# Anaesthesiaye/sound_event_detection_transformer

Hardware: AMD Instinct MI355X
Metric: audio clips/sec training throughput (B=64, 10s@64-mel) (higher is better)
Workload: dtype bf16; 1 GPU; URBAN-SED SEDT enc_layers=3 dec_at num_queries=10 B=64/GPU, 10 s @ 64-mel (B,1,500,64), full train step: fwd + Hungarian matching (device) + SetCriterion + bwd + clip 0.1 + AdamW, dropout 0.1; global_batch=64, parallelism=dp1

## Files before the change

### include/sedt_hip.h

```cpp
#ifndef SEDT_HIP_H
#define SEDT_HIP_H
#include <stddef.h>
#include <stdint.h>

#ifdef __cplusplus
extern "C" {
#endif

#define SEDT_F32 0
#define SEDT_BF16 1
#define SEDT_BF16X3 2

#define SEDT_ACT_NONE 0
#define SEDT_ACT_RELU 1
#define SEDT_ACT_SIGMOID 2

const char* sedt_last_error(void);
int sedt_version(void);

typedef struct SedtIgemm {
  int32_t M, N, K;
  const void* A;
  const void* B;
  int64_t lda, ldb;
// ... 19 lines not shown
  float* slab;
  int32_t tile_m, tile_n;
  float* colsum_out;
  uint8_t* bits_out;
  int64_t ldbits;
  int32_t mask_bits;
  int32_t f32ep;
  int32_t omap;
  int32_t o_Hi, o_Wi, o_sh, o_sw, o_h0, o_w0;
  int32_t btap_on;
  int32_t btap[8];
  void* split_out;
  int32_t awrap;
  int32_t pad2_;
  const void* bfrag;
} SedtIgemm;

int sedt_igemm(const SedtIgemm* args, int dtype, void* stream);
int sedt_sizeof(int which);
int sedt_igemm_group(const SedtIgemm* jobs, int njobs, int dtype, void* stream);
int sedt_wgrad_group(const SedtIgemm* jobs, int njobs, int dtype, void* stream);
int sedt_igemm_co(const SedtIgemm* main, const SedtIgemm* wjobs, int nw, int dtype, void* stream, int* taken);
int sedt_igemm_splitk(int M, int N, int K, int dtype);
int sedt_igemm_describe(const SedtIgemm* args, int dtype, int grouped, char* out, int cap);
int sedt_igemm_group_describe(const SedtIgemm* jobs, int njobs, int dtype, char* out, int cap);

int sedt_wgrad_reduce(const float* slab, int splitk, int R, int taps, int Ci, const float* rowscale,
                      float* out, void* stream);
int sedt_wgrad_reduce_bias(const float* slab, int splitk, int R, int taps, int Ci, const float* rowscale, float* out,
                           const float* colsum_slab, float* bias_out, void* stream);

typedef struct SedtPrefetch {
  const void* ptr[3];
  size_t bytes[3];
} SedtPrefetch;

typedef struct SedtSplitJob {
  const float* src;
  int64_t ld;
  void* dst;
  int32_t rows, cols, pattern;
  int32_t blk0;
} SedtSplitJob;
int sedt_split3(const SedtSplitJob* jobs, int njobs, void* stream);

#define SEDT_MAX_REDUCE_JOBS 40
// ... 324 lines not shown
```

### sound_event_detection_transformer_amd/csrc/host.cpp

```cpp
#include <math.h>
#include <stdint.h>
#include <vector>
#include "../../include/sedt_hip.h"

namespace sedt { void set_error(const char* fmt, ...); }

template <typename F>
static void lsa_rows_le_cols(int n, int m, F a, std::vector<int>& row_of_col) {
  const double INF = 1e300;
  std::vector<double> u(n + 1, 0.0), v(m + 1, 0.0), minv(m + 1);
  std::vector<int> p(m + 1, 0), way(m + 1, 0);
  std::vector<char> used(m + 1);
  for (int i = 1; i <= n; ++i) {
    p[0] = i;
    int j0 = 0;
    std::fill(minv.begin(), minv.end(), INF);
    std::fill(used.begin(), used.end(), 0);
    do {
      used[j0] = 1;
      int i0 = p[j0], j1 = 0;
      double delta = INF;
      for (int j = 1; j <= m; ++j) {
        if (used[j]) continue;
        double cur = a(i0 - 1, j - 1) - u[i0] - v[j];
// ... 44 lines not shown
        lsa_rows_le_cols(Q, n, [&](int q, int t) { return (double)c[(size_t)q * Nt + t]; }, roc);
        for (int t = 0; t < n; ++t)
          if (roc[t] >= 0) out[roc[t]] = t;
      }
    }
  }
  return 0;
}

extern "C" int sedt_sizeof(int which) {
  switch (which) {
    case 0: return (int)sizeof(SedtIgemm);
    case 1: return (int)sizeof(SedtReduceJob);
    case 2: return (int)sizeof(SedtSplitJob);
    case 3: return (int)sizeof(SedtPrefetch);
    case 4: return (int)sizeof(SedtCriterion);
    case 5: return (int)sizeof(SedtMatch);
    case 6: return (int)sizeof(SedtChunk);
    case 7: return (int)sizeof(SedtBnJob);
    case 8: return (int)sizeof(SedtPackJob);
    case 9: return (int)sizeof(SedtFragJob);
    case 10: return (int)sizeof(SedtPoolAt);
    case 11: return (int)sizeof(SedtCopyJob);
    default: return -1;
  }
}
```

### sound_event_detection_transformer_amd/csrc/igemm.hip

```cpp
#include <stdlib.h>
#include "common.h"

namespace sedt {

template <typename T> struct Cfg;
template <> struct Cfg<float> {
  static constexpr int BK = 32, PITCH = 33, EPC = 4, KSTEP = 2, UK = 1;
};
template <> struct Cfg<bf16_t> {
  static constexpr int BK = 64, PITCH = 72, EPC = 8, KSTEP = 16, UK = 4;
};

struct GatherGeom {
  int Hi, Wi, Ci, Ho, Wo, KH, KW, sh, sw, ph, pw, dh, dw, transposed;
};

__device__ __forceinline__ long gather_pix(const GatherGeom& g, int n, int ho, int wo, int kh, int kw) {
  int hi, wi;
  if (!g.transposed) {
    hi = ho * g.sh - g.ph + kh * g.dh;
    wi = wo * g.sw - g.pw + kw * g.dw;
    if ((unsigned)hi >= (unsigned)g.Hi || (unsigned)wi >= (unsigned)g.Wi) return -1;
  } else {
    int th = ho + g.ph - kh * g.dh, tw = wo + g.pw - kw * g.dw;
// ... 698 lines not shown
  int maxs = nkb / 4 > 1 ? nkb / 4 : 1;
  if (s > maxs) s = maxs;
  if (s > 128) s = 128;
  if (tiles <= 2) s = maxs < 512 ? maxs : 512;
  if (s < 1) s = 1;
  static int kslice = -1;
  if (kslice < 0) {
    const char* e = sedt::dev_getenv("SEDT_WGRAD_KSLICE");
    kslice = (e && e[0] == '1') ? 1 : 0;
  }
  if (kslice && dtype == SEDT_BF16) {
    const int taps = (N % 9 == 0 && (N / 9) % 64 == 0) ? 9 : 1;
    const double A = 2.0 * K * M, B = 2.0 * K * (N / taps);
    const double cur = (N > M ? 8.0 * A + B : A + 8.0 * B) + 2.0 * s * 4.0 * M * N;
    int s8 = ((s + 7) / 8) * 8;
    if (s8 < 8) s8 = 8;
    if (s8 <= maxs && s8 <= 128) {
      const double ks = A + B + 2.0 * s8 * 4.0 * M * N;
      if (ks < 0.8 * cur) s = s8;
    }
  }
  return s;
}
```

### sound_event_detection_transformer_amd/csrc/wgrad3.hip

```cpp
#include <stdlib.h>
#include <algorithm>
#include "wgrad3_body.h"

namespace sedt {

template <int BN>
__global__ __launch_bounds__(256) void wgrad3_kernel(const SedtIgemm p, const unsigned a_bytes, const unsigned b_bytes,
                                                     const int nmajor) {
  wgrad3_body<BN>(p, a_bytes, b_bytes, nmajor, blockIdx.x, blockIdx.y);
}

__global__ __launch_bounds__(256) void wgrad3_group_kernel(const WgradGroup g) { wgrad_group_run(g, blockIdx.x); }

template <int BN>
static int launch_wgrad3(const SedtIgemm& p, unsigned a_bytes, unsigned b_bytes, hipStream_t st) {
  SEDT_DESCRIBE("wgrad3_kernel<%d>", BN);
  constexpr size_t lds = (size_t)2 * (64 * ROWB + 64 * BN * 2);
  static bool attr_set = false;
  auto kern = wgrad3_kernel<BN>;
  if (!attr_set) {
    hipError_t e = hipFuncSetAttribute(reinterpret_cast<const void*>(kern), hipFuncAttributeMaxDynamicSharedMemorySize, (int)lds);
    if (e != hipSuccess) {
      set_error("wgrad3: hipFuncSetAttribute failed: %s", hipGetErrorString(e));
      return 1;
// ... 30 lines not shown
  long ab[WG_MAXG], bb[WG_MAXG];
  for (int base = 0; base < njobs; base += WG_MAXG) {
    const int n = std::min(WG_MAXG, njobs - base);
    for (int i = 0; i < n; ++i) {
      const SedtIgemm& p = jobs[base + i];
      if (!p.trans || wgrad_lds_envelope(p, &ab[i], &bb[i]) != 0 || !wgrad3_conv_ok(p)) return -1;
    }
  }
  static bool attr_set = false;
  constexpr size_t lds = (size_t)2 * (64 * ROWB + 64 * 64 * 2);
  if (!attr_set) {
    hipError_t e = hipFuncSetAttribute(reinterpret_cast<const void*>(wgrad3_group_kernel), hipFuncAttributeMaxDynamicSharedMemorySize,
                                       (int)lds);
    if (e != hipSuccess) {
      set_error("wgrad3 group: hipFuncSetAttribute failed: %s", hipGetErrorString(e));
      return 1;
    }
    attr_set = true;
  }
  for (int base = 0; base < njobs; base += WG_MAXG) {
    WgradGroup g, gw;
    g.n = gw.n = 0;
    const int n = std::min(WG_MAXG, njobs - base);
    int blk = 0;
    for (int j = 0; j < n; ++j) {
      const SedtIgemm& p = jobs[base + j];
      long a, b;
      wgrad_lds_envelope(p, &a, &b);
      if (wgrad4_ok(p)) {
        const int i = gw.n++;
        gw.p[i] = p;
        gw.a_bytes[i] = (unsigned)a;
        gw.b_bytes[i] = (unsigned)b;
        continue;
      }
      const int i = g.n++;
      g.p[i] = p;
      g.a_bytes[i] = (unsigned)a;
      g.b_bytes[i] = (unsigned)b;
      g.nwg[i] = ((p.N + 63) / 64) * ((p.M + 63) / 64);
      g.nmajor[i] = (p.N > p.M ? 1 : 0) + ((p.splitk >= 8 && p.splitk % 8 == 0) ? 2 : 0);
      g.blk0[i] = blk;
      blk += (g.nwg[i] * (p.splitk > 1 ? p.splitk : 1) + 7) / 8 * 8;
    }
    if (gw.n > 0)
      if (int r = launch_wgrad4_group(gw, st)) return r;
    if (g.n > 0) {
      g.blk0[g.n] = blk;
      hipLaunchKernelGGL(wgrad3_group_kernel, dim3(blk), dim3(256), lds, st, g);
// ... 50 lines not shown
  if ((p.M & 7) || (p.N & 7) || (p.lda & 7) || (p.ldb & 7)) return -1;
  if (!al16(p.A) || !al16(p.B)) return -1;
  if (p.conv && ((p.Ci & 7) || p.transposed)) return -1;
  long a_bytes = ((long)(p.K - 1) * p.lda + p.M) * 2;
  long b_rows = p.conv ? (long)((p.K + (long)p.Ho * p.Wo - 1) / ((long)p.Ho * p.Wo)) * p.Hi * p.Wi : (long)p.K;
  long b_bytes = ((b_rows - 1) * p.ldb + (p.conv ? p.Ci : p.N)) * 2;
  if (a_bytes >= (1L << 31) || b_bytes >= (1L << 31) || a_bytes <= 0 || b_bytes <= 0) return -1;
  *a_bytes_out = a_bytes;
  *b_bytes_out = b_bytes;
  return 0;
}

int wgrad_lds_try(const SedtIgemm& p, hipStream_t st) {
  long a_bytes, b_bytes;
  if (wgrad_lds_envelope(p, &a_bytes, &b_bytes) != 0) return -1;
  {
    int r3 = wgrad3_try(p, (unsigned)a_bytes, (unsigned)b_bytes, st);
    if (r3 >= 0) return r3;
  }
  return -1;
}

}
```

### sound_event_detection_transformer_amd/csrc/wgrad3_body.h

```cpp
#pragma once
#include "lds_gemm_common.h"

namespace sedt {

typedef __attribute__((ext_vector_type(4))) short w3_s16x4;
typedef __attribute__((ext_vector_type(8))) short w3_s16x8;
typedef __attribute__((address_space(3))) w3_s16x4 w3_lds_s16x4;

__device__ __forceinline__ int w3_uniform(int v) { return __builtin_amdgcn_readfirstlane(v); }

__device__ __forceinline__ int w3_swz(int row) {
  const int v = (row >> 1) & 7;
  return ((v & 1) << 2) | (v & 2) | (v >> 2);
}

template <int BN, bool CONV>
__device__ __forceinline__ void wgrad3_impl(const SedtIgemm& p, const unsigned a_bytes, const unsigned b_bytes, const int nmajor,
                                            const int bx, const int by) {
  constexpr int BM = 64, BKP = 64;
  constexpr int NI = BN / 64;
  constexpr int A_BYTES = BKP * ROWB;
  constexpr int B_ROWB = BN * 2;
  constexpr int STAGE_BYTES = A_BYTES + BKP * B_ROWB;
  constexpr int GA = 2, GB = BN / 32;
// ... 197 lines not shown
  float* out = p.splitk > 1 ? p.slab + (long)by * p.M * p.N : reinterpret_cast<float*>(p.C);
  const long ldo = p.splitk > 1 ? p.N : p.ldc;
#pragma unroll
  for (int j = 0; j < NI; ++j) {
    const int col = n0 + wn + j * 32 + (lane & 31);
    if (col < p.N) {
#pragma unroll
      for (int r = 0; r < 16; ++r) {
        const int row = m0 + wm + (r & 3) + 8 * (r >> 2) + 4 * (lane >> 5);
        if (row < p.M) out[(long)row * ldo + col] = acc[j][r];
      }
    }
  }
}

template <int BN>
__device__ __forceinline__ void wgrad3_body(const SedtIgemm& p, const unsigned a_bytes, const unsigned b_bytes, const int nmajor,
                                            const int bx, const int by) {
  if (p.conv) wgrad3_impl<BN, true>(p, a_bytes, b_bytes, nmajor, bx, by);
  else wgrad3_impl<BN, false>(p, a_bytes, b_bytes, nmajor, bx, by);
}

constexpr int WG_MAXG = 10;
struct WgradGroup {
  int n;
  int blk0[WG_MAXG + 1];
  int nwg[WG_MAXG];
  int nmajor[WG_MAXG];
  unsigned a_bytes[WG_MAXG], b_bytes[WG_MAXG];
  SedtIgemm p[WG_MAXG];
};

static_assert(sizeof(WgradGroup) <= 3900, "WgradGroup must fit the 4 KB kernel-argument segment");

__device__ __forceinline__ void wgrad_group_run(const WgradGroup& g, const int b) {
  int i = 0;
  while (i + 1 < g.n && b >= g.blk0[i + 1]) ++i;
  const int local = b - g.blk0[i];
  const int nwg = g.nwg[i], sk = g.p[i].splitk > 1 ? g.p[i].splitk : 1;
  if (local >= nwg * sk) return;
  if (g.nmajor[i] >= 2) {
    const int j = local >> 3;
    wgrad3_body<64>(g.p[i], g.a_bytes[i], g.b_bytes[i], g.nmajor[i], j % nwg, (local & 7) + 8 * (j / nwg));
  } else {
    wgrad3_body<64>(g.p[i], g.a_bytes[i], g.b_bytes[i], g.nmajor[i], local % nwg, local / nwg);
  }
}

}
```

### sound_event_detection_transformer_amd/csrc/wgrad4.hip

```cpp
#include <stdlib.h>
#include <algorithm>
#include "wgrad3_body.h"

namespace sedt {

__device__ __forceinline__ int w4_swz(int row) { return (row & 3) << 2; }

template <bool CONV, int S, int NA>
__device__ __forceinline__ void wgrad4_impl(const SedtIgemm& p, const unsigned a_bytes, const unsigned b_bytes, const int nmajor,
                                            const int bx, const int by) {
  constexpr int BM = 128 * NA, BN = 128, BKP = 64, NW = 8;
  constexpr int IMG_ROWB = 256;
  constexpr int IMG_BYTES = BKP * IMG_ROWB;
  constexpr int STAGE_BYTES = (NA + 1) * IMG_BYTES;
  constexpr int B_IMG = NA * IMG_BYTES;
  constexpr int CPR = 16, RPI = 4;
  constexpr int GB = BKP / RPI / NW, GA = NA * GB;
  constexpr int G = GA + GB;
  constexpr int MI = 2 * NA;
  constexpr unsigned OOB = 0x80000000u;
  extern __shared__ __attribute__((aligned(16))) unsigned char smem[];
  const int t = threadIdx.x, lane = t & 63;
  const int wave = w3_uniform(t >> 6);
  const int kgrp = wave >> 2;
// ... 275 lines not shown
  if (nmajor & 2) {
    if (p.conv) wgrad4_impl<true, 3, 2>(p, a_bytes, b_bytes, nmajor, bx, by);
    else wgrad4_impl<false, 3, 2>(p, a_bytes, b_bytes, nmajor, bx, by);
    return;
  }
  if (p.conv) wgrad4_impl<true, S, 1>(p, a_bytes, b_bytes, nmajor, bx, by);
  else wgrad4_impl<false, S, 1>(p, a_bytes, b_bytes, nmajor, bx, by);
}

template <int S>
__global__ __launch_bounds__(512) void wgrad4_kernel(const SedtIgemm p, const unsigned a_bytes, const unsigned b_bytes,
                                                     const int nmajor) {
  wgrad4_body<S>(p, a_bytes, b_bytes, nmajor, blockIdx.x, blockIdx.y);
}

template <int S>
__global__ __launch_bounds__(512) void wgrad4_group_kernel(const WgradGroup g) {
  const int b = blockIdx.x;
  int i = 0;
  while (i + 1 < g.n && b >= g.blk0[i + 1]) ++i;
  const int local = b - g.blk0[i];
  const int nwg = g.nwg[i], sk = g.p[i].splitk > 1 ? g.p[i].splitk : 1;
  if (local >= nwg * sk) return;
  wgrad4_body<S>(g.p[i], g.a_bytes[i], g.b_bytes[i], g.nmajor[i], local % nwg, local / nwg);
}

static int wg4_stages() {
  static int s = -1;
  if (s < 0) {
    const char* e = sedt::dev_getenv("SEDT_WGRAD4_STAGES");
    s = (e && atoi(e) == 3) ? 3 : (e && atoi(e) == 4) ? 4 : 3;
  }
  return s;
}
int wgrad4_tile_m(int M, int N) {
  static int bm = -1, min_tiles = 1;
  if (bm < 0) {
    const char* e = sedt::dev_getenv("SEDT_WGRAD4_BM");
    bm = (e && atoi(e) == 128) ? 128 : 256;
    e = sedt::dev_getenv("SEDT_WGRAD4_WIDE_MIN");
    min_tiles = e ? atoi(e) : 1;
  }
  return (bm == 256 && M % 256 == 0 && (long)(M / 256) * (N / 128) >= min_tiles) ? 256 : 128;
}
static size_t wg4_lds() {
  const size_t narrow = (size_t)wg4_stages() * 2 * 64 * 256, wide = (size_t)3 * 3 * 64 * 256;
  return wgrad4_tile_m(256, 1 << 20) == 256 ? std::max(narrow, wide) : narrow;
}

bool wgrad4_shape_ok(int M, int N) {
  static int mn = -1;
  if (mn < 0) {
    const char* e = sedt::dev_getenv("SEDT_WGRAD4_MIN");
    mn = e ? atoi(e) : 256;
  }
  return M >= mn && N >= mn && (M % 128) == 0 && (N % 128) == 0;
}

bool wgrad4_ok(const SedtIgemm& p) {
  static int on = -1;
  if (on < 0) {
    const char* e = sedt::dev_getenv("SEDT_WGRAD_V4");
    on = (e && e[0] == '0') ? 0 : 1;
  }
  static int with_bias = -1;
  if (with_bias < 0) {
    const char* e = sedt::dev_getenv("SEDT_WGRAD4_BIAS");
    with_bias = (e && e[0] == '1') ? 1 : 0;
  }
  return on && p.trans && wgrad4_shape_ok(p.M, p.N) && (p.colsum_out == nullptr || with_bias) && p.out_f32 &&
         (p.splitk > 1 ? p.slab != nullptr : ((p.ldc & 3) == 0 && (reinterpret_cast<uintptr_t>(p.C) & 15) == 0)) &&
         (reinterpret_cast<uintptr_t>(p.slab) & 15) == 0;
}

static bool wg4_cbmajor(const SedtIgemm& p) {
  static int on = -1;
  if (on < 0) {
    const char* e = sedt::dev_getenv("SEDT_WGRAD4_CBMAJOR");
    on = e ? atoi(e) : 1;
  }
  return on && p.conv && p.KH * p.KW > 1 && (p.Ci % 128) == 0 && p.N == p.KH * p.KW * p.Ci;
}

template <typename K>
static int wg4_attr(K kern, const char* what) {
  hipError_t e = hipFuncSetAttribute(reinterpret_cast<const void*>(kern), hipFuncAttributeMaxDynamicSharedMemorySize, (int)wg4_lds());
  if (e != hipSuccess) {
    set_error("%s: hipFuncSetAttribute failed: %s", what, hipGetErrorString(e));
    return 1;
  }
  return 0;
}

// ... 14 lines not shown
}

int launch_wgrad4_group(WgradGroup& g, hipStream_t st) {
  static bool attr_set = false;
  if (!attr_set) {
    if (wg4_attr(wgrad4_group_kernel<3>, "wgrad4 group") || wg4_attr(wgrad4_group_kernel<4>, "wgrad4 group")) return 1;
    attr_set = true;
  }
  int blk = 0;
  for (int i = 0; i < g.n; ++i) {
    const SedtIgemm& p = g.p[i];
    const int bm = wgrad4_tile_m(p.M, p.N);
    g.nwg[i] = (p.N / 128) * (p.M / bm);
    g.nmajor[i] = (p.N > p.M ? 1 : 0) | (bm == 256 ? 2 : 0) | (wg4_cbmajor(p) ? 4 : 0);
    g.blk0[i] = blk;
    blk += (g.nwg[i] * (p.splitk > 1 ? p.splitk : 1) + 7) / 8 * 8;
  }
  g.blk0[g.n] = blk;
  if (wg4_stages() == 4) hipLaunchKernelGGL(wgrad4_group_kernel<4>, dim3(blk), dim3(512), wg4_lds(), st, g);
  else hipLaunchKernelGGL(wgrad4_group_kernel<3>, dim3(blk), dim3(512), wg4_lds(), st, g);
  return check_launch("wgrad4_group");
}

}
```

### sound_event_detection_transformer_amd/lib.py

```python
import ctypes as C
import os

import torch

HERE = os.path.dirname(os.path.abspath(__file__))
LIB_PATH = os.path.join(HERE, 'libsedt_hip.so')
if os.environ.get('SEDT_LIB_AB') and os.environ.get('SEDT_DEV') == '1':
    LIB_PATH = os.environ['SEDT_LIB_AB']

F32, BF16 = 0, 1
BF16X3 = 2
GEMM_X3 = False


def gemm_dtype(dtype):
    return BF16X3 if (dtype == F32 and GEMM_X3) else dtype
ACT_NONE, ACT_RELU, ACT_SIGMOID = 0, 1, 2
TORCH_DTYPE = {F32: torch.float32, BF16: torch.bfloat16}


class SedtIgemm(C.Structure):
    _fields_ = [
        ('M', C.c_int32), ('N', C.c_int32), ('K', C.c_int32),
        ('A', C.c_void_p), ('B', C.c_void_p),
# ... 45 lines not shown
POOL_MODES = {'max': 0, 'avg': 1, 'attn': 2, 'weighted_sum': 3}


class SedtMatch(C.Structure):
    _fields_ = [(n, C.c_void_p) for n in ('logits', 'boxes', 'lab_cat', 'lab_off', 'box_cat', 'box_off', 'ratio_cat', 'tc',
                                           'coef', 'wbox', 'tbox', 'tidx', 'tgt_len', 'gt_weak', 'assign')] + \
               [(n, C.c_int32) for n in ('L', 'B', 'ns', 'Q', 'C', 'n_lab', 'max_targets')] + \
               [('layer_of', C.c_int32 * CRIT_MAXL), ('w_class', C.c_float), ('w_bbox', C.c_float), ('w_giou', C.c_float),
                ('fl', C.c_int32), ('fine_tune', C.c_int32), ('normalize', C.c_int32), ('alpha_fl', C.c_float),
                ('gamma_fl', C.c_float), ('epsilon', C.c_float), ('alpha', C.c_float), ('ft_rand', C.c_void_p),
                ('ft_seed', C.c_uint32), ('seed_ptr', C.c_void_p), ('split', C.c_void_p), ('Qs', C.c_int32), ('q0', C.c_int32)]


class SedtSplitJob(C.Structure):
    _fields_ = [('src', C.c_void_p), ('ld', C.c_int64), ('dst', C.c_void_p), ('rows', C.c_int32), ('cols', C.c_int32),
                ('pattern', C.c_int32), ('blk0', C.c_int32)]


class SedtCopyJob(C.Structure):
    _fields_ = [('src', C.c_void_p), ('dst', C.c_void_p), ('src_stride', C.c_int64), ('dst_stride', C.c_int64), ('outer', C.c_int32),
                ('inner', C.c_int32), ('blk0', C.c_int32), ('pad_', C.c_int32)]


class SedtPrefetch(C.Structure):
    _fields_ = [('ptr', C.c_void_p * 3), ('bytes', C.c_size_t * 3)]


def prefetch_arg(tensors):
    ts = [t for t in (tensors or ()) if t is not None][:3]
    if not ts:
        return None
    a = SedtPrefetch()
    for i, t in enumerate(ts):
        a.ptr[i], a.bytes[i] = t.data_ptr(), t.numel() * t.element_size()
    return C.byref(a)


MAX_REDUCE_JOBS = 40
_vp, _i, _i64, _f, _d, _u32, _sz = C.c_void_p, C.c_int, C.c_int64, C.c_float, C.c_double, C.c_uint32, C.c_size_t

SIGNATURES = {
    'sedt_last_error': (C.c_char_p, []),
    'sedt_version': (_i, []),
    'sedt_sizeof': (_i, [_i]),
    'sedt_igemm': (_i, [C.POINTER(SedtIgemm), _i, _vp]),
    'sedt_igemm_group': (_i, [C.POINTER(SedtIgemm), _i, _i, _vp]),
    'sedt_wgrad_group': (_i, [C.POINTER(SedtIgemm), _i, _i, _vp]),
    'sedt_igemm_co': (_i, [C.POINTER(SedtIgemm), C.POINTER(SedtIgemm), _i, _i, _vp, C.POINTER(C.c_int)]),
    'sedt_igemm_splitk': (_i, [_i, _i, _i, _i]),
    'sedt_igemm_describe': (_i, [C.POINTER(SedtIgemm), _i, _i, C.c_char_p, _i]),
    'sedt_igemm_group_describe': (_i, [C.POINTER(SedtIgemm), _i, _i, C.c_char_p, _i]),
    'sedt_wgrad_reduce': (_i, [_vp, _i, _i, _i, _i, _vp, _vp, _vp]),
    'sedt_wgrad_reduce_bias': (_i, [_vp, _i, _i, _i, _i, _vp, _vp, _vp, _vp, _vp]),
    'sedt_split3': (_i, [C.POINTER(SedtSplitJob), _i, _vp]),
    'sedt_copy2d': (_i, [C.POINTER(SedtCopyJob), _i, _vp]),
    'sedt_multi_wgrad_reduce': (_i, [C.POINTER(SedtReduceJob), _i, C.POINTER(SedtPrefetch), _vp]),
    'sedt_skinny_linear_fwd': (_i, [_vp, _i64, _vp, _vp, _vp, _i64, _i, _i, _i, _i, _i, _i, _vp]),
    'sedt_skinny_linear_bwd_scratch': (_sz, [_i]),
    'sedt_skinny_linear_bwd': (_i, [_vp, _vp, _i64, _vp, _vp, _i64, _vp, _i64, _vp, _i64, _vp, _vp, _vp, _i, _i, _i, _i, _i, _i, _vp]),
    'sedt_colsum': (_i, [_vp, _i64, _i, _i, _i, _i, _vp, _vp, _sz, _vp]),
    'sedt_colsum_scratch': (_sz, [_i, _i]),
    'sedt_dropout_grad': (_i, [_vp, _i64, _vp, _i64, _i, _i, _f, _u32, _vp, _i, _vp]),
    'sedt_add': (_i, [_vp, _vp, _vp, _i, _i, _i, _i, _vp]),
    'sedt_add_n': (_i, [C.POINTER(C.c_void_p), _i, _vp, _i64, _i, _vp]),
    'sedt_cast': (_i, [_vp, _i, _vp, _i, _i64, _vp]),
    'sedt_relu_mask': (_i, [_vp, _vp, _vp, _i64, _i, _vp]),
    'sedt_spsedt_dec_in': (_i, [_vp, _vp, _vp, _vp, _vp, _i, _i, _i, _i, _i, _i, _f, _u32, _vp, _i, _vp]),
    'sedt_spsedt_dec_in_bwd': (_i, [_vp, _vp, _vp, _vp, _i, _i, _i, _i, _i, _i, _i, _vp]),
    'sedt_gelu_fwd': (_i, [_vp, _vp, _i64, _f, _u32, _vp, _i, _vp]),
    'sedt_gelu_bwd': (_i, [_vp, _vp, _vp, _i64, _f, _u32, _vp, _i, _vp]),
    'sedt_sigmoid_grad': (_i, [_vp, _vp, _vp, _i64, _vp]),
    'sedt_layernorm_fwd': (_i, [_vp, _vp, _vp, _vp, _vp, _vp, _vp, _vp, _i, _i, _i, _vp]),
# ... 123 lines not shown
```

### sound_event_detection_transformer_amd/ops.py

```python
import ctypes as C

import os
import numpy as np
import torch

from . import lib as L
from .lib import F32, BF16, ACT_NONE, ACT_RELU, ACT_SIGMOID, TORCH_DTYPE, p as _p


class ConvGeom(object):
    __slots__ = ('Hi', 'Wi', 'Ci', 'Ho', 'Wo', 'Co', 'KH', 'KW', 'sh', 'sw', 'ph', 'pw', 'dh', 'dw')

    def __init__(self, Hi, Wi, Ci, Co, k=1, stride=1, pad=0, dil=1):
        self.Hi, self.Wi, self.Ci, self.Co = Hi, Wi, Ci, Co
        self.KH = self.KW = k
        self.sh = self.sw = stride
        self.ph = self.pw = pad
        self.dh = self.dw = dil
        self.Ho = (Hi + 2 * pad - dil * (k - 1) - 1) // stride + 1
        self.Wo = (Wi + 2 * pad - dil * (k - 1) - 1) // stride + 1

    @property
    def taps(self):
        return self.KH * self.KW
# ... 568 lines not shown
    def add_gemm(self, dtype, args, shape, code=None):
        self.group.append((args, shape, L.gemm_dtype(dtype) if code is None else code))
        self.group_dtype = dtype

    def _launch_group(self):
        if not self.group:
            return
        lib = L.load()
        if PROFILE is not None:
            for a, shape, code in self.group:
                L.check(lib.sedt_igemm(C.byref(a), code, L.stream_ptr()), 'sedt_igemm')
                PROFILE.append((a, code, shape, (list(self.keep), list(self.operands)), 'wgrad_group'))
        else:
            i = 0
            while i < len(self.group):
                j = i
                while j < len(self.group) and self.group[j][2] == self.group[i][2]:
                    j += 1
                arr = (L.SedtIgemm * (j - i))(*[g[0] for g in self.group[i:j]])
                L.check(lib.sedt_wgrad_group(arr, j - i, self.group[i][2], L.stream_ptr()), 'wgrad_group')
                i = j
        self.group = []

    def defer(self, body, operands):
        self.deferred.append(body)
        self.operands.extend(t for t in operands if t is not None)

    def add(self, slab, sk, R, taps, Ci, rowscale, out, cs, bias_out, cs_splitk=0):
        j = L.SedtReduceJob()
        j.slab, j.out, j.splitk, j.R, j.taps, j.Ci = slab.data_ptr(), out.data_ptr(), sk, R, taps, Ci
        j.cs_splitk = cs_splitk
        j.rowscale = rowscale.data_ptr() if rowscale is not None else None
        j.colsum_slab = cs.data_ptr() if cs is not None else None
        j.bias_out = bias_out.data_ptr() if (cs is not None and bias_out is not None) else None
        self.jobs.append(j)
        self.keep.append((slab, cs, rowscale, None, None) if self.shared else (slab, cs, rowscale, out, bias_out))
        if len(self.jobs) == L.MAX_REDUCE_JOBS and not _co['on'] and not self.shared:
            self._launch_group()
            self._launch()

    def add_colsum(self, partial, nrows, ncols, out):
        j = L.SedtReduceJob()
        j.colsum_slab, j.bias_out, j.splitk, j.R, j.taps, j.Ci = partial.data_ptr(), out.data_ptr(), nrows, ncols, 1, 0
        self.jobs.append(j)
        self.keep.append((partial, None, None, None if self.shared else out, None))

    def _launch(self):
        for i in range(0, len(self.jobs), L.MAX_REDUCE_JOBS):
            chunk = self.jobs[i:i + L.MAX_REDUCE_JOBS]
            arr = (L.SedtReduceJob * len(chunk))(*chunk)
            pf = None
            if self.prefetch is not None and RED_PREFETCH and i + L.MAX_REDUCE_JOBS >= len(self.jobs):
                pf = L.prefetch_arg(self.prefetch)
            L.check(L.load().sedt_multi_wgrad_reduce(arr, len(chunk), pf, L.stream_ptr()), 'multi_wgrad_reduce')
        self.jobs, self.keep = [], []

    prefetch = None

    def collect(self):
        for body in self.deferred:
            body()
        self.deferred = []

    def flush(self, prefetch=None):
        from . import runtime
        self.prefetch = prefetch
        if _co['on'] and not runtime.async_wgrad_on():
            for body in self.deferred:
                body()
            self.deferred = []
            if self.group_dtype in (None, BF16):
                POOL.push(self.group, BF16, self.jobs, [k[:3] for k in self.keep], self.operands)
                self.group, self.jobs, self.keep, self.operands = [], [], [], []
                return
        if self.deferred:
            with runtime.side(*self.operands):
                for body in self.deferred:
                    body()
                self._launch_group()
                self._launch()
            self.deferred, self.operands = [], []
        else:
            self._launch_group()
            self._launch()


DEFER_LAYER_WGRADS = _dev_env('SEDT_DEFER_LAYER_WGRADS', '1') != '0'
_defer = {'on': False}


class defer_layer_wgrads(object):

    def __init__(self, enable=True):
        self.enable = bool(enable) and DEFER_LAYER_WGRADS

    def __enter__(self):
        self.prev = _defer['on']
        _defer['on'] = self.enable
        return self

    def __exit__(self, *exc):
        _defer['on'] = self.prev
        return False


class WgradShare(object):

    def __init__(self):
        self.rb = None
        self.mark = 0
# ... 42 lines not shown
        global GRAD_SINK
        GRAD_SINK = self.prev
        return False


def _sink(param, shape):
    if GRAD_SINK is None or param is None:
        return None
    v = GRAD_SINK.pop(param.data_ptr(), None)
    return v.view(shape) if v is not None and v.numel() == int(np.prod(shape)) else None


def _x3_wgrad_ok(dy, x, g, B):
    if not X3_FAST or dy.dtype != torch.float32 or x.dtype != torch.float32:
        return False
    Co, Ci = g.Co, g.Ci
    if Co % 8 or Ci % 8 or dy.stride(0) % 4 or x.stride(0) % 4 or dy.data_ptr() % 16 or x.data_ptr() % 16:
        return False
    if not g.plain and ((64 % g.Wo) != 0 or g.Ho * g.Wo < 64 or g.Ho < 64 // g.Wo):
        return False
    return B * g.Ho * g.Wo * 3 * Co * 2 < (1 << 31) and B * g.Hi * g.Wi * 3 * Ci * 2 < (1 << 31)


def wgrad(dtype, dy, x, B, g, rowscale=None, out=None, bias_out=None, batch=None, param=None):
    from . import runtime
    lib = L.load()
    Mo, No, Kp = g.Co, g.taps * g.Ci, B * g.Ho * g.Wo
    sk = lib.sedt_igemm_splitk(Mo, No, Kp, dtype)
    own_out = False
    if out is None:
        out = _sink(param, (g.Co, g.Ci, g.KH, g.KW))
        if out is None:
            out = torch.empty((g.Co, g.Ci, g.KH, g.KW), device=dy.device, dtype=torch.float32)
            own_out = True

    def body():
        conv = None if g.plain else _geom_tuple(g)
        if dtype == F32 and L.GEMM_X3 and _x3_wgrad_ok(dy, x, g, B):
            sk3 = max(1, lib.sedt_igemm_splitk(2 * Mo, No, Kp, BF16))
            rows_x = B * g.Hi * g.Wi
            dy3, x3 = _split3([(dy, 0, Kp, Mo, dy.stride(0), 0), (x, 0, rows_x, g.Ci, x.stride(0), 0)])
            slab = torch.empty((3 * sk3, Mo, No), device=dy.device, dtype=torch.float32)
            cs = torch.empty((2 * sk3, Mo), device=dy.device, dtype=torch.float32) if bias_out is not None else None
            a1 = igemm_args(2 * Mo, No, Kp, dy3, 2 * Mo, x3, 2 * g.Ci, slab, No, trans=1, conv=conv, out_f32=1, splitk=sk3, slab=slab,
                            colsum_out=cs)
            x3lo, slab2 = x3[:, g.Ci:2 * g.Ci], slab[2 * sk3:]
            a2 = igemm_args(Mo, No, Kp, dy3, 2 * Mo, x3lo, 2 * g.Ci, slab2, No, trans=1, conv=conv, out_f32=1, splitk=sk3, slab=slab2)
            tb = batch if batch is not None else ReduceBatch()
            tb.add_gemm(dtype, a1, (2 * Mo, No, Kp, 1, 0 if conv is None else 1), code=BF16)
            tb.add_gemm(dtype, a2, (Mo, No, Kp, 1, 0 if conv is None else 1), code=BF16)
            tb.add(slab, 3 * sk3, Mo, g.taps, g.Ci, rowscale, out, cs, bias_out, cs_splitk=2 * sk3)
            tb.keep.append((dy3, x3, None, None, None))
            if batch is None:
                tb._launch_group()
                tb._launch()
            return
        slab = torch.empty((sk, Mo, No), device=dy.device, dtype=torch.float32)
        fused = bias_out is not None and _fused_bias_ok(dtype, dy, x, g)
        cs = torch.empty((sk, Mo), device=dy.device, dtype=torch.float32) if fused else None
        if batch is not None:
            batch.add_gemm(dtype, igemm_args(Mo, No, Kp, dy, dy.stride(0), x, x.stride(0), slab, No, trans=1, conv=conv,
                                             out_f32=1, splitk=sk, slab=slab, colsum_out=cs),
                           (Mo, No, Kp, 1, 0 if conv is None else 1))
            batch.add(slab, sk, Mo, g.taps, g.Ci, rowscale, out, cs, bias_out if fused else None)
        else:
            igemm(dtype, Mo, No, Kp, dy, dy.stride(0), x, x.stride(0), slab, No, trans=1, conv=conv, out_f32=1, splitk=sk,
                  slab=slab, colsum_out=cs)
            L.check(lib.sedt_wgrad_reduce_bias(_p(slab), sk, Mo, g.taps, g.Ci, _p(rowscale), _p(out), _p(cs),
                                               _p(bias_out) if fused else None, L.stream_ptr()), 'wgrad_reduce')
        if bias_out is not None and not fused:
            colsum(dtype, dy, out=bias_out)

    if batch is not None:
        batch.defer(body, (dy, x, rowscale))
        if batch.shared and param is not None and own_out and tuple(param.shape) == tuple(out.shape[:param.dim()]):
            batch.expect.append((param, out.data_ptr()))
    else:
        with runtime.side(dy, x, rowscale):
            body()
    return out


def linear_wgrad(dtype, dy, x, out=None, bias_out=None, batch=None, param=None):
    N, K = dy.shape[1], x.shape[1]
    g = ConvGeom(1, 1, K, N)
    return wgrad(dtype, dy, x, dy.shape[0], g, out=out.view(N, K, 1, 1) if out is not None else None,
                 bias_out=bias_out, batch=batch, param=param).view(N, K)


def colsum(dtype, x, out=None):
    lib = L.load()
    rows, cols = x.shape
    if out is None:
        out = torch.empty((cols,), device=x.device, dtype=torch.float32)
    nb = lib.sedt_colsum_scratch(rows, cols)
    scratch = torch.empty((max(nb // 4, 1),), device=x.device, dtype=torch.float32)
    L.check(lib.sedt_colsum(_p(x), x.stride(0), rows, cols, int(x.dtype == torch.float32), dtype, _p(out), _p(scratch),
# ... 801 lines not shown
```

Before: 12450 clips/s.

## Plan per-job split-k across grouped wgrad launches with a makespan cost model

```diff
diff --git a/include/sedt_hip.h b/include/sedt_hip.h
--- a/include/sedt_hip.h
+++ b/include/sedt_hip.h
@@ -65,6 +65,15 @@
 int sedt_wgrad_group(const SedtIgemm* jobs, int njobs, int dtype, void* stream);
 int sedt_igemm_co(const SedtIgemm* main, const SedtIgemm* wjobs, int nw, int dtype, void* stream, int* taken);
 int sedt_igemm_splitk(int M, int N, int K, int dtype);
+typedef struct SedtWgradShape {
+  int32_t M, N, K;
+  int32_t bias;
+  int32_t solo;
+  int32_t fixed;
+} SedtWgradShape;
+int sedt_wgrad_group_plan(const SedtWgradShape* probs, int n, int dtype, int* splitk_out);
+int sedt_wgrad_group_cost(const SedtWgradShape* probs, int n, int dtype, const int* splitk, int longest_first, double* makespan_us,
+                          double* slab_bytes);
 int sedt_igemm_describe(const SedtIgemm* args, int dtype, int grouped, char* out, int cap);
 int sedt_igemm_group_describe(const SedtIgemm* jobs, int njobs, int dtype, char* out, int cap);
 
diff --git a/sound_event_detection_transformer_amd/csrc/host.cpp b/sound_event_detection_transformer_amd/csrc/host.cpp
--- a/sound_event_detection_transformer_amd/csrc/host.cpp
+++ b/sound_event_detection_transformer_amd/csrc/host.cpp
@@ -90,6 +90,7 @@
     case 9: return (int)sizeof(SedtFragJob);
     case 10: return (int)sizeof(SedtPoolAt);
     case 11: return (int)sizeof(SedtCopyJob);
+    case 12: return (int)sizeof(SedtWgradShape);
     default: return -1;
   }
 }
diff --git a/sound_event_detection_transformer_amd/csrc/igemm.hip b/sound_event_detection_transformer_amd/csrc/igemm.hip
--- a/sound_event_detection_transformer_amd/csrc/igemm.hip
+++ b/sound_event_detection_transformer_amd/csrc/igemm.hip
@@ -1,4 +1,10 @@
 #include <stdlib.h>
+#include <algorithm>
+#include <functional>
+#include <map>
+#include <mutex>
+#include <tuple>
+#include <vector>
 #include "common.h"
 
 namespace sedt {
@@ -744,3 +750,220 @@
   }
   return s;
 }
+
+namespace sedt {
+bool wgrad4_route(int M, int N, bool fused_bias);
+
+struct WgForm { double kt_us, kt_mapped_us, fixed_us; int resident; };
+static const WgForm WG_FORM[3] = {{1.34, 1.05, 4.0, 3}, {0.57, 0.57, 13.0, 1}, {0.85, 0.85, 13.0, 1}};
+static const double WG_SLAB_BYTES_PER_US = 5.0e6;
+static const int WG_CUS = 256;
+
+struct WgProb {
+  int form, tiles, nkb, count;
+  double mn;
+};
+struct WgRun { double cost; long count; };
+
+static int wg_form(const SedtWgradShape& q) {
+  if (!wgrad4_route(q.M, q.N, q.bias != 0)) return 0;
+  return wgrad4_tile_m(q.M, q.N) == 256 ? 2 : 1;
+}
+static int wg_tiles(const SedtWgradShape& q, int form) {
+  if (form == 0) return ((q.M + 63) / 64) * ((q.N + 63) / 64);
+  return (q.M / (form == 2 ? 256 : 128)) * (q.N / 128);
+}
+static int wg_canonical(int nkb, int s) {
+  if (s <= 1) return 1;
+  const int per = (nkb + s - 1) / s;
+  return (nkb + per - 1) / per;
+}
+
+static void wg_add_runs(std::vector<WgRun>& runs, const WgProb& q, int s) {
+  const WgForm& f = WG_FORM[q.form];
+  if (s < 1) s = 1;
+  const double kt_us = (s >= 8 && s % 8 == 0) ? f.kt_mapped_us : f.kt_us;
+  const int per = (q.nkb + s - 1) / s, used = (q.nkb + per - 1) / per, last = q.nkb - (used - 1) * per;
+  const long tiles = (long)q.tiles * q.count;
+  if (used > 1) runs.push_back({kt_us * per + f.fixed_us, tiles * (used - 1)});
+  runs.push_back({kt_us * last + f.fixed_us, tiles});
+  if (s > used) runs.push_back({f.fixed_us, tiles * (s - used)});
+}
+
+static double wg_makespan(const std::vector<WgRun>& runs, int slots) {
+  long items = 0;
+  for (const WgRun& r : runs) items += r.count;
+  if (items == 0) return 0.0;
+  std::vector<double> heap((size_t)std::min<long>(slots, items), 0.0);
+  const auto later = std::greater<double>();
+  double end = 0.0;
+  for (const WgRun& r : runs)
+    for (long k = 0; k < r.count; ++k) {
+      std::pop_heap(heap.begin(), heap.end(), later);
+      const double t = heap.back() + r.cost;
+      heap.back() = t;
+      std::push_heap(heap.begin(), heap.end(), later);
+      if (t > end) end = t;
+    }
+  return end;
+}
+
+static double wg_chunk_makespan(const std::vector<WgProb>& probs, const std::vector<int>& split, bool longest_first) {
+  double total = 0.0;
+  for (int launch = 0; launch < 2; ++launch) {
+    std::vector<WgRun> runs;
+    if (longest_first) {
+      std::vector<int> order;
+      for (size_t i = 0; i < probs.size(); ++i)
+        if ((probs[i].form == 0) == (launch == 0)) order.push_back((int)i);
+      auto per = [&](int i) { const int sk = std::max(1, split[i]); return (probs[i].nkb + sk - 1) / sk; };
+      std::stable_sort(order.begin(), order.end(), [&](int a, int b) { return per(a) > per(b); });
+      for (int i : order) wg_add_runs(runs, probs[i], split[i]);
+    } else {
+      for (size_t i = 0; i < probs.size(); ++i)
+        if ((probs[i].form == 0) == (launch == 0)) wg_add_runs(runs, probs[i], split[i]);
+    }
+    total += wg_makespan(runs, WG_CUS * WG_FORM[launch == 0 ? 0 : 2].resident);
+  }
+  return total;
+}
+
+static double wg_slab_us(const std::vector<WgProb>& probs, const std::vector<int>& split) {
+  double bytes = 0.0;
+  for (size_t i = 0; i < probs.size(); ++i) bytes += 2.0 * std::max(1, split[i]) * probs[i].mn * 4.0 * probs[i].count;
+  return bytes / WG_SLAB_BYTES_PER_US;
+}
+
+static void wg_plan_chunk(const SedtWgradShape* q, int n, int* out) {
+  struct Cls { int M, N, K, bias, fixed, base; bool locked; };
+  std::vector<Cls> cls;
+  std::vector<int> cls_of(n);
+  for (int i = 0; i < n; ++i) {
+    const int base = sedt_igemm_splitk(q[i].M, q[i].N, q[i].K, SEDT_BF16);
+    Cls c = {q[i].M, q[i].N, q[i].K, q[i].bias != 0, q[i].fixed > 0 ? q[i].fixed : 0, base, false};
+    c.locked = c.fixed > 0 || (long)((c.M + 63) / 64) * ((c.N + 63) / 64) <= 2;
+    if (c.fixed > 0) c.base = c.fixed;
+    cls.push_back(c);
+  }
+  auto key_less = [](const Cls& a, const Cls& b) {
+    return std::make_tuple(a.M, a.N, a.K, a.bias, a.fixed) < std::make_tuple(b.M, b.N, b.K, b.bias, b.fixed);
+  };
+  auto key_eq = [&](const Cls& a, const Cls& b) { return !key_less(a, b) && !key_less(b, a); };
+  std::vector<Cls> uniq = cls;
+  std::sort(uniq.begin(), uniq.end(), key_less);
+  uniq.erase(std::unique(uniq.begin(), uniq.end(), key_eq), uniq.end());
+  const int nc = (int)uniq.size();
+  std::vector<WgProb> probs(nc);
+  for (int c = 0; c < nc; ++c) {
+    SedtWgradShape sh = {uniq[c].M, uniq[c].N, uniq[c].K, uniq[c].bias, 0, 0};
+    const int form = wg_form(sh);
+    probs[c] = {form, wg_tiles(sh, form), (uniq[c].K + 63) / 64, 0, (double)uniq[c].M * uniq[c].N};
+  }
+  for (int i = 0; i < n; ++i) {
+    cls_of[i] = (int)(std::lower_bound(uniq.begin(), uniq.end(), cls[i], key_less) - uniq.begin());
+    probs[cls_of[i]].count++;
+  }
+  std::vector<int> base(nc);
+  for (int c = 0; c < nc; ++c) base[c] = uniq[c].base;
+  const double base_mk = wg_chunk_makespan(probs, base, true);
+  auto total = [&](const std::vector<int>& s, double* mk) {
+    *mk = wg_chunk_makespan(probs, s, true);
+    return *mk + wg_slab_us(probs, s);
+  };
+  static const int CAND[] = {1, 2, 3, 4, 5, 6, 7, 8, 10, 12, 14, 16, 20, 24, 28, 32, 40, 48, 56, 64, 80, 96, 112, 128};
+  auto descend = [&](std::vector<int> s, bool keep_makespan, double* cost_out, double* mk_out) {
+    double mk, best = total(s, &mk);
+    for (int pass = 0; pass < 6; ++pass) {
+      bool moved = false;
+      for (int c = 0; c < nc; ++c) {
+        if (uniq[c].locked) continue;
+        const int maxs = std::max(1, std::min(128, probs[c].nkb / 4));
+        int prev = 0;
+        for (int cand : CAND) {
+          if (cand > maxs) break;
+          const int v = wg_canonical(probs[c].nkb, cand);
+          if (v == prev || v == s[c]) { prev = v; continue; }
+          prev = v;
+          const int old = s[c];
+          s[c] = v;
+          double m;
+          const double t = total(s, &m);
+          if (t < best - 1e-9 && (!keep_makespan || m <= base_mk + 1e-9)) { best = t; mk = m; moved = true; }
+          else s[c] = old;
+        }
+      }
+      if (!moved) break;
+    }
+    *cost_out = best;
+    *mk_out = mk;
+    return s;
+  };
+  double cost_a, mk_a, cost_b, mk_b;
+  std::vector<int> a = descend(base, true, &cost_a, &mk_a);
+  std::vector<int> ones = base;
+  for (int c = 0; c < nc; ++c)
+    if (!uniq[c].locked) ones[c] = 1;
+  std::vector<int> b = descend(ones, false, &cost_b, &mk_b);
+  const std::vector<int>& pick = (mk_b <= base_mk + 1e-9 && cost_b < cost_a - 1e-9) ? b : a;
+  for (int i = 0; i < n; ++i) out[i] = pick[cls_of[i]];
+}
+
+static bool wg_plan_applies(const SedtWgradShape* q, int n, int dtype) {
+  if (dtype != SEDT_BF16 || n < 2) return false;
+  for (int i = 0; i < n; ++i)
+    if (q[i].solo) return false;
+  return true;
+}
+}
+
+extern "C" int sedt_wgrad_group_plan(const SedtWgradShape* probs, int n, int dtype, int* splitk_out) {
+  using namespace sedt;
+  SEDT_REQUIRE(probs && splitk_out && n >= 1, "wgrad_group_plan: bad arguments");
+  for (int i = 0; i < n; ++i) {
+    SEDT_REQUIRE(probs[i].M >= 1 && probs[i].N >= 1 && probs[i].K >= 1, "wgrad_group_plan: bad shape");
+    splitk_out[i] = probs[i].fixed > 0 ? probs[i].fixed : sedt_igemm_splitk(probs[i].M, probs[i].N, probs[i].K, dtype);
+  }
+  if (!wg_plan_applies(probs, n, dtype)) return 0;
+  static std::mutex mu;
+  static std::map<std::vector<int>, std::vector<int>> memo;
+  std::vector<int> key;
+  for (int i = 0; i < n; ++i) key.insert(key.end(), {probs[i].M, probs[i].N, probs[i].K, probs[i].bias != 0, probs[i].fixed > 0 ? probs[i].fixed : 0});
+  std::lock_guard<std::mutex> lock(mu);
+  auto it = memo.find(key);
+  if (it == memo.end()) {
+    std::vector<int> plan(n);
+    for (int base = 0; base < n; base += WG_MAXG) {
+      const int m = std::min(WG_MAXG, n - base);
+      if (m >= 2) wg_plan_chunk(probs + base, m, plan.data() + base);
+      else plan[base] = splitk_out[base];
+    }
+    it = memo.emplace(key, plan).first;
+  }
+  std::copy(it->second.begin(), it->second.end(), splitk_out);
+  return 0;
+}
+
+extern "C" int sedt_wgrad_group_cost(const SedtWgradShape* probs, int n, int dtype, const int* splitk, int longest_first,
+                                     double* makespan_us, double* slab_bytes) {
+  using namespace sedt;
+  SEDT_REQUIRE(probs && splitk && n >= 1 && makespan_us && slab_bytes, "wgrad_group_cost: bad arguments");
+  SEDT_REQUIRE(dtype == SEDT_BF16, "wgrad_group_cost: the model covers the bf16 grouped launches only");
+  double mk = 0.0, bytes = 0.0;
+  for (int base = 0; base < n; base += WG_MAXG) {
+    const int m = std::min(WG_MAXG, n - base);
+    std::vector<WgProb> ps(m);
+    std::vector<int> s(m);
+    for (int i = 0; i < m; ++i) {
+      const SedtWgradShape& q = probs[base + i];
+      SEDT_REQUIRE(q.M >= 1 && q.N >= 1 && q.K >= 1 && splitk[base + i] >= 1, "wgrad_group_cost: bad shape or factor");
+      const int form = wg_form(q);
+      ps[i] = {form, wg_tiles(q, form), (q.K + 63) / 64, 1, (double)q.M * q.N};
+      s[i] = splitk[base + i];
+      if (s[i] > 1) bytes += (double)s[i] * q.M * q.N * 4.0;
+    }
+    mk += wg_chunk_makespan(ps, s, longest_first != 0);
+  }
+  *makespan_us = mk;
+  *slab_bytes = bytes;
+  return 0;
+}
diff --git a/sound_event_detection_transformer_amd/csrc/wgrad3.hip b/sound_event_detection_transformer_amd/csrc/wgrad3.hip
--- a/sound_event_detection_transformer_amd/csrc/wgrad3.hip
+++ b/sound_event_detection_transformer_amd/csrc/wgrad3.hip
@@ -76,9 +76,19 @@
     WgradGroup g, gw;
     g.n = gw.n = 0;
     const int n = std::min(WG_MAXG, njobs - base);
+    int order[WG_MAXG];
+    for (int j = 0; j < n; ++j) order[j] = j;
+    static int longest_first = -1;
+    if (longest_first < 0) {
+      const char* e = sedt::dev_getenv("SEDT_WGRAD_LONGEST_FIRST");
+      longest_first = (e && e[0] == '0') ? 0 : 1;
+    }
+    if (longest_first)
+      std::stable_sort(order, order + n,
+                       [&](int a, int b) { return wgrad_item_ktiles(jobs[base + a]) > wgrad_item_ktiles(jobs[base + b]); });
     int blk = 0;
     for (int j = 0; j < n; ++j) {
-      const SedtIgemm& p = jobs[base + j];
+      const SedtIgemm& p = jobs[base + order[j]];
       long a, b;
       wgrad_lds_envelope(p, &a, &b);
       if (wgrad4_ok(p)) {
@@ -175,3 +185,26 @@
 }
 
 }
+
+#ifdef SEDT_DEV
+namespace sedt {
+int wg_ts_set4(WgTsBuf* buf);
+static WgTsBuf* wg_ts_buf = nullptr;
+}
+extern "C" int sedt_dev_wg_ts_reset() {
+  using namespace sedt;
+  if (wg_ts_buf == nullptr) {
+    if (hipMalloc(reinterpret_cast<void**>(&wg_ts_buf), sizeof(WgTsBuf)) != hipSuccess) return 1;
+    if (hipMemcpyToSymbol(HIP_SYMBOL(wg_ts_dev), &wg_ts_buf, sizeof(wg_ts_buf)) != hipSuccess || wg_ts_set4(wg_ts_buf)) return 1;
+  }
+  return hipMemset(wg_ts_buf, 0, 32) == hipSuccess && hipDeviceSynchronize() == hipSuccess ? 0 : 1;
+}
+extern "C" int sedt_dev_wg_ts_read(void* out, int cap) {
+  using namespace sedt;
+  unsigned n = 0;
+  if (wg_ts_buf == nullptr || hipDeviceSynchronize() != hipSuccess || hipMemcpy(&n, wg_ts_buf, 4, hipMemcpyDeviceToHost) != hipSuccess) return -1;
+  const unsigned m = std::min(std::min(n, WG_TS_CAP), (unsigned)std::max(cap, 0));
+  if (m > 0 && hipMemcpy(out, wg_ts_buf->rec, (size_t)m * sizeof(WgTsRec), hipMemcpyDeviceToHost) != hipSuccess) return -1;
+  return (int)std::min(n, WG_TS_CAP);
+}
+#endif
diff --git a/sound_event_detection_transformer_amd/csrc/wgrad3_body.h b/sound_event_detection_transformer_amd/csrc/wgrad3_body.h
--- a/sound_event_detection_transformer_amd/csrc/wgrad3_body.h
+++ b/sound_event_detection_transformer_amd/csrc/wgrad3_body.h
@@ -243,6 +243,12 @@
 }
 
 constexpr int WG_MAXG = 10;
+#ifdef SEDT_DEV
+struct WgTsRec { unsigned long long t0, t1; unsigned cu, blocks, prob, ktiles, M, N, form, pad_; };
+constexpr unsigned WG_TS_CAP = 1u << 16;
+struct WgTsBuf { unsigned n, pad_[7]; WgTsRec rec[WG_TS_CAP]; };
+static __device__ WgTsBuf* wg_ts_dev = nullptr;
+#endif
 struct WgradGroup {
   int n;
   int blk0[WG_MAXG + 1];
@@ -252,6 +258,36 @@
   SedtIgemm p[WG_MAXG];
 };
 
+__host__ __device__ inline int wgrad_item_ktiles(const SedtIgemm& p) {
+  const int nkb = (p.K + 63) / 64, sk = p.splitk > 1 ? p.splitk : 1;
+  return (nkb + sk - 1) / sk;
+}
+
+#ifdef SEDT_DEV
+#define WG_TS_BEGIN() const unsigned long long wg_ts_t0_ = __builtin_amdgcn_s_memrealtime()
+#define WG_TS_END(g_, i_, by_, form_)                                                                         \
+  do {                                                                                                        \
+    if (wg_ts_dev != nullptr && threadIdx.x == 0) {                                                                  \
+      const SedtIgemm& q_ = (g_).p[i_];                                                                       \
+      const int nkb_ = (q_.K + 63) / 64, per_ = wgrad_item_ktiles(q_);                                        \
+      const int kt_ = max(0, min(nkb_, ((by_) + 1) * per_) - (by_) * per_);                                   \
+      const unsigned hw_ = __builtin_amdgcn_s_getreg((31 << 11) | 4), xcc_ = __builtin_amdgcn_s_getreg((31 << 11) | 20); \
+      const unsigned k_ = atomicAdd(&wg_ts_dev->n, 1u);                                                       \
+      if (k_ < WG_TS_CAP) {                                                                                   \
+        WgTsRec r_;                                                                                           \
+        r_.t0 = wg_ts_t0_; r_.t1 = __builtin_amdgcn_s_memrealtime();                                          \
+        r_.cu = ((xcc_ & 15u) << 8) | ((hw_ >> 8) & 255u);                                                    \
+        r_.blocks = (unsigned)gridDim.x; r_.prob = (unsigned)(i_); r_.ktiles = (unsigned)kt_;               \
+        r_.M = (unsigned)q_.M; r_.N = (unsigned)q_.N; r_.form = (unsigned)(form_); r_.pad_ = 0;               \
+        wg_ts_dev->rec[k_] = r_;                                                                              \
+      }                                                                                                       \
+    }                                                                                                         \
+  } while (0)
+#else
+#define WG_TS_BEGIN() do {} while (0)
+#define WG_TS_END(g_, i_, by_, form_) do {} while (0)
+#endif
+
 static_assert(sizeof(WgradGroup) <= 3900, "WgradGroup must fit the 4 KB kernel-argument segment");
 
 __device__ __forceinline__ void wgrad_group_run(const WgradGroup& g, const int b) {
@@ -260,12 +296,15 @@
   const int local = b - g.blk0[i];
   const int nwg = g.nwg[i], sk = g.p[i].splitk > 1 ? g.p[i].splitk : 1;
   if (local >= nwg * sk) return;
+  WG_TS_BEGIN();
   if (g.nmajor[i] >= 2) {
     const int j = local >> 3;
     wgrad3_body<64>(g.p[i], g.a_bytes[i], g.b_bytes[i], g.nmajor[i], j % nwg, (local & 7) + 8 * (j / nwg));
+    WG_TS_END(g, i, (local & 7) + 8 * (j / nwg), 0);
   } else {
     wgrad3_body<64>(g.p[i], g.a_bytes[i], g.b_bytes[i], g.nmajor[i], local % nwg, local / nwg);
-  }
-}
-
-}
+    WG_TS_END(g, i, local / nwg, 0);
+  }
+}
+
+}
diff --git a/sound_event_detection_transformer_amd/csrc/wgrad4.hip b/sound_event_detection_transformer_amd/csrc/wgrad4.hip
--- a/sound_event_detection_transformer_amd/csrc/wgrad4.hip
+++ b/sound_event_detection_transformer_amd/csrc/wgrad4.hip
@@ -321,7 +321,9 @@
   const int local = b - g.blk0[i];
   const int nwg = g.nwg[i], sk = g.p[i].splitk > 1 ? g.p[i].splitk : 1;
   if (local >= nwg * sk) return;
+  WG_TS_BEGIN();
   wgrad4_body<S>(g.p[i], g.a_bytes[i], g.b_bytes[i], g.nmajor[i], local % nwg, local / nwg);
+  WG_TS_END(g, i, local / nwg, (g.nmajor[i] & 2) ? 2 : 1);
 }
 
 static int wg4_stages() {
@@ -356,7 +358,7 @@
   return M >= mn && N >= mn && (M % 128) == 0 && (N % 128) == 0;
 }
 
-bool wgrad4_ok(const SedtIgemm& p) {
+bool wgrad4_route(int M, int N, bool fused_bias) {
   static int on = -1;
   if (on < 0) {
     const char* e = sedt::dev_getenv("SEDT_WGRAD_V4");
@@ -367,7 +369,11 @@
     const char* e = sedt::dev_getenv("SEDT_WGRAD4_BIAS");
     with_bias = (e && e[0] == '1') ? 1 : 0;
   }
-  return on && p.trans && wgrad4_shape_ok(p.M, p.N) && (p.colsum_out == nullptr || with_bias) && p.out_f32 &&
+  return on && wgrad4_shape_ok(M, N) && (!fused_bias || with_bias);
+}
+
+bool wgrad4_ok(const SedtIgemm& p) {
+  return p.trans && wgrad4_route(p.M, p.N, p.colsum_out != nullptr) && p.out_f32 &&
          (p.splitk > 1 ? p.slab != nullptr : ((p.ldc & 3) == 0 && (reinterpret_cast<uintptr_t>(p.C) & 15) == 0)) &&
          (reinterpret_cast<uintptr_t>(p.slab) & 15) == 0;
 }
@@ -428,4 +434,8 @@
   return check_launch("wgrad4_group");
 }
 
-}
+#ifdef SEDT_DEV
+int wg_ts_set4(WgTsBuf* buf) { return hipMemcpyToSymbol(HIP_SYMBOL(wg_ts_dev), &buf, sizeof(buf)) == hipSuccess ? 0 : 1; }
+#endif
+
+}
diff --git a/sound_event_detection_transformer_amd/lib.py b/sound_event_detection_transformer_amd/lib.py
--- a/sound_event_detection_transformer_amd/lib.py
+++ b/sound_event_detection_transformer_amd/lib.py
@@ -91,6 +91,10 @@
                 ('inner', C.c_int32), ('blk0', C.c_int32), ('pad_', C.c_int32)]
 
 
+class SedtWgradShape(C.Structure):
+    _fields_ = [(n, C.c_int32) for n in ('M', 'N', 'K', 'bias', 'solo', 'fixed')]
+
+
 class SedtPrefetch(C.Structure):
     _fields_ = [('ptr', C.c_void_p * 3), ('bytes', C.c_size_t * 3)]
 
@@ -117,6 +121,8 @@
     'sedt_wgrad_group': (_i, [C.POINTER(SedtIgemm), _i, _i, _vp]),
     'sedt_igemm_co': (_i, [C.POINTER(SedtIgemm), C.POINTER(SedtIgemm), _i, _i, _vp, C.POINTER(C.c_int)]),
     'sedt_igemm_splitk': (_i, [_i, _i, _i, _i]),
+    'sedt_wgrad_group_plan': (_i, [C.POINTER(SedtWgradShape), _i, _i, C.POINTER(C.c_int)]),
+    'sedt_wgrad_group_cost': (_i, [C.POINTER(SedtWgradShape), _i, _i, C.POINTER(C.c_int), _i, C.POINTER(C.c_double), C.POINTER(C.c_double)]),
     'sedt_igemm_describe': (_i, [C.POINTER(SedtIgemm), _i, _i, C.c_char_p, _i]),
     'sedt_igemm_group_describe': (_i, [C.POINTER(SedtIgemm), _i, _i, C.c_char_p, _i]),
     'sedt_wgrad_reduce': (_i, [_vp, _i, _i, _i, _i, _vp, _vp, _vp]),
diff --git a/sound_event_detection_transformer_amd/ops.py b/sound_event_detection_transformer_amd/ops.py
--- a/sound_event_detection_transformer_amd/ops.py
+++ b/sound_event_detection_transformer_amd/ops.py
@@ -614,9 +614,28 @@
                 i = j
         self.group = []
 
-    def defer(self, body, operands):
-        self.deferred.append(body)
+    def defer(self, body, operands, shape=None):
+        self.deferred.append((body, shape))
         self.operands.extend(t for t in operands if t is not None)
+
+    def _run_deferred(self):
+        shaped = [sh for _, sh in self.deferred if sh is not None]
+        plan = []
+        if shaped:
+            lib = L.load()
+            if _co['on'] or not GROUP_PLAN:
+                plan = [sh.fixed if sh.fixed > 0 else lib.sedt_igemm_splitk(sh.M, sh.N, sh.K, BF16) for sh in shaped]
+            else:
+                arr, out = (L.SedtWgradShape * len(shaped))(*shaped), (C.c_int * len(shaped))()
+                L.check(lib.sedt_wgrad_group_plan(arr, len(shaped), BF16, out), 'wgrad_group_plan')
+                plan = list(out)
+        plan.reverse()
+        for body, sh in self.deferred:
+            if sh is None:
+                body()
+            else:
+                body(plan.pop())
+        self.deferred = []
 
     def add(self, slab, sk, R, taps, Ci, rowscale, out, cs, bias_out, cs_splitk=0):
         j = L.SedtReduceJob()
@@ -650,34 +669,30 @@
     prefetch = None
 
     def collect(self):
-        for body in self.deferred:
-            body()
-        self.deferred = []
+        self._run_deferred()
 
     def flush(self, prefetch=None):
         from . import runtime
         self.prefetch = prefetch
         if _co['on'] and not runtime.async_wgrad_on():
-            for body in self.deferred:
-                body()
-            self.deferred = []
+            self._run_deferred()
             if self.group_dtype in (None, BF16):
                 POOL.push(self.group, BF16, self.jobs, [k[:3] for k in self.keep], self.operands)
                 self.group, self.jobs, self.keep, self.operands = [], [], [], []
                 return
         if self.deferred:
             with runtime.side(*self.operands):
-                for body in self.deferred:
-                    body()
+                self._run_deferred()
                 self._launch_group()
                 self._launch()
-            self.deferred, self.operands = [], []
+            self.operands = []
         else:
             self._launch_group()
             self._launch()
 
 
 DEFER_LAYER_WGRADS = _dev_env('SEDT_DEFER_LAYER_WGRADS', '1') != '0'
+GROUP_PLAN = _dev_env('SEDT_WGRAD_GROUP_PLAN', '1') != '0'
 _defer = {'on': False}
 
 
@@ -766,11 +781,23 @@
     return B * g.Ho * g.Wo * 3 * Co * 2 < (1 << 31) and B * g.Hi * g.Wi * 3 * Ci * 2 < (1 << 31)
 
 
-def wgrad(dtype, dy, x, B, g, rowscale=None, out=None, bias_out=None, batch=None, param=None):
+def _wgrad_shape(dtype, dy, x, g, Mo, No, Kp, bias_out, splitk):
+    if dtype != BF16:
+        return None
+    sh = L.SedtWgradShape()
+    sh.M, sh.N, sh.K = Mo, No, Kp
+    lds = _fused_bias_ok(dtype, dy, x, g)
+    sh.bias = 1 if (bias_out is not None and lds) else 0
+    sh.solo = 0 if (lds and (g.plain or (64 % g.Wo == 0 and g.Ho * g.Wo >= 64 and g.Ho >= 64 // g.Wo))) else 1
+    sh.fixed = splitk or 0
+    return sh
+
+
+def wgrad(dtype, dy, x, B, g, rowscale=None, out=None, bias_out=None, batch=None, param=None, splitk=None):
     from . import runtime
     lib = L.load()
     Mo, No, Kp = g.Co, g.taps * g.Ci, B * g.Ho * g.Wo
-    sk = lib.sedt_igemm_splitk(Mo, No, Kp, dtype)
+    shape = _wgrad_shape(dtype, dy, x, g, Mo, No, Kp, bias_out, splitk) if batch is not None else None
     own_out = False
     if out is None:
         out = _sink(param, (g.Co, g.Ci, g.KH, g.KW))
@@ -778,7 +805,9 @@
             out = torch.empty((g.Co, g.Ci, g.KH, g.KW), device=dy.device, dtype=torch.float32)
             own_out = True
 
-    def body():
+    def body(sk=None):
+        if sk is None:
+            sk = splitk or lib.sedt_igemm_splitk(Mo, No, Kp, dtype)
         conv = None if g.plain else _geom_tuple(g)
         if dtype == F32 and L.GEMM_X3 and _x3_wgrad_ok(dy, x, g, B):
             sk3 = max(1, lib.sedt_igemm_splitk(2 * Mo, No, Kp, BF16))
@@ -816,7 +845,7 @@
             colsum(dtype, dy, out=bias_out)
 
     if batch is not None:
-        batch.defer(body, (dy, x, rowscale))
+        batch.defer(body, (dy, x, rowscale), shape=shape)
         if batch.shared and param is not None and own_out and tuple(param.shape) == tuple(out.shape[:param.dim()]):
             batch.expect.append((param, out.data_ptr()))
     else:
```

Result: no change. 12540 clips/s (median of 6 runs) (+0.7%).
